# RichealYoung/BRIEF_PyTorch

Measured on AMD Instinct MI355X. Metric: encode_voxels_per_sec, higher is better.
Workload: dtype f32; 1 GPU; SingleTask 512^3 synthetic uint16 volume, SIREN 4x256 (layers=5, features=256, w0=20), randompoint sample_size=100000, datal2, Adamax lr=1e-3; layers=5, features=256, sample_size=100000, params=198657

## Files before the change

### brief_pytorch_amd/csrc/brief_hip.hip

```cpp
#include <hip/hip_runtime.h>
#include <hip/hip_ext.h>
#include <stdint.h>
#include <stdio.h>
#include <string.h>
#include <stdlib.h>
#include <mutex>
#include "brief_layout.h"
#include "brief_math.h"

#include "brief_device.inc"
#include "brief_fused.inc"
#include "brief_lean.inc"
#include "brief_wide.inc"
#include "brief_small.inc"
#include "brief_wgrad.inc"
#include "brief_x3.inc"
#include "brief_reduce.inc"
#include "brief_bf16.inc"
#include "brief_aux.inc"
#include "brief_ffn.inc"
#include "brief_nerf.inc"
#include "brief_mfn.inc"

static thread_local char g_err[512] = "";
// ... 829 lines not shown
            const int lds_big = (int)(sizeof(float) * 4 * W16B_PANEL);
            if (int rc = dev_attr_once((const void *)k_wgrad16_big, lds_big)) return rc;
            if (ov.on) {
                wa.kb_lo = 0; wa.kb_hi = ov.kb_body; wa.split_lo = 0; wa.nsplit_here = ov.na;
                hipLaunchKernelGGL(k_wgrad16_big, dim3((hidden * ov.na + 7) / 8 * 8 * 4), dim3(512), lds_big, st, wa);
                wa.kb_lo = ov.kb_body; wa.kb_hi = np / 64; wa.split_lo = ov.na; wa.nsplit_here = 1;
                hipLaunchKernelGGL(k_wgrad16_big, dim3((hidden + 7) / 8 * 8 * 4), dim3(512), lds_big, side, wa);
            } else {
                const int groups8 = (hidden * nsp + 7) / 8 * 8;
                hipLaunchKernelGGL(k_wgrad16_big, dim3(groups8 * 4), dim3(512), lds_big, st, wa);
            }
        } else if (hidden > 0) {
            hipLaunchKernelGGL(k_wgrad16<false>, dim3(hidden * nb * nb * nsp), dim3(256), sizeof(float) * 4 * W16_PANEL, st, wa);
        }
        hipLaunchKernelGGL(k_wgrad16<true>, dim3((wa.bias_jobs ? hidden * nb * nsp : 0) + 2 * nb * nsp_s), dim3(256), sizeof(float) * 4 * W16_PANEL, side, wa);
        HIP_TRY(hipGetLastError());
        if (ov.on) {
            HIP_TRY(hipEventRecord(dev_state()->aux_join, side));
            HIP_TRY(hipStreamWaitEvent(st, dev_state()->aux_join, 0));
        }
        const int64_t l0c = (int64_t)d->features * d->cin + d->features;
        const int64_t hcnt = brief_canon_head_off(*d) - l0c;
        if (hidden > 0) {
            ReduceArgs ra;
            memset(&ra, 0, sizeof(ra));
            ra.d = *d; ra.slabs = ws + w16.slabs; ra.nsplit = nsp; ra.sgroups = 1;
            ra.grads = grads; ra.loss_out = loss_out; ra.inv_count = inv16;
            if (upd) { ra.update = 1; ra.opt = upd->opt; ra.params = upd->params; ra.s1 = upd->s1; ra.s2 = upd->s2; ra.pk = upd->pk; }
            ra.sgroups = 1;
            const int nbh = (int)((hcnt + 255) / 256);
            hipLaunchKernelGGL(k_reduce, dim3(nbh), dim3(256), 0, st, ra, nbh);
            HIP_TRY(hipGetLastError());
        }
        Reduce16Args r16;
        memset(&r16, 0, sizeof(r16));
        r16.d = *d; r16.slabs = ws + w16.slabs + (int64_t)hidden * nsp * (FP * FP + FP); r16.nsplit = nsp_s;
        r16.rec = fa.rec; r16.nwg = g16; r16.grads = grads; r16.loss_out = loss_out; r16.inv_count = inv16;
        if (upd) { r16.update = 1; r16.opt = upd->opt; r16.params = upd->params; r16.s1 = upd->s1; r16.s2 = upd->s2; r16.pk = upd->pk; }
        const int64_t items = l0c + (int64_t)d->cout * d->features + d->cout + 1;
        hipLaunchKernelGGL(k_reduce16, dim3((unsigned)((items + 3) / 4)), dim3(256), 0, st, r16);
        HIP_TRY(hipGetLastError());
        return 0;
    }
    const bool small = use_small(*d);
    const FusedPlan fp = fused_plan(*d, batch->n, true);
    TailPlan tp;
    memset(&tp, 0, sizeof(tp));
    if (!small) tp = fused_tail_plan(*d, batch->n);
    const int grid1 = small ? small_grid(*d, batch->n) : (tp.on ? tp.grid_body + tp.grid_tail : fp.grid);
    const int nsplit = small ? (d->layers > 2 ? grid1 : 0) : wgrad_splits(*d, batch->n);
    const float inv_count = (float)(1.0 / ((double)batch->n * d->cout));

    FusedArgs fa;
    memset(&fa, 0, sizeof(fa));
    fa.d = *d; fa.pk = packed;
    fa.coords = batch->coords; fa.targets = batch->targets; fa.weights = batch->weights;
    fa.idx = batch->idx; fa.offset = batch->offset; fa.n = batch->n;
    if (!batch->idx && batch->rng_pop > 0) { fa.rng_pop = (uint64_t)batch->rng_pop; fa.rng_seed = batch->rng_seed; fa.rng_step = batch->rng_step; }
    fill_grid(fa.grid, grid);
    fa.loss_kind = loss_kind; fa.thr = thr; fa.beta = beta; fa.inv_count = inv_count;
    fa.Z = ws + wl.z; fa.D = ws + wl.dd; fa.npad = brief_npad_d(*d, batch->n);
    fa.rec = ws + wl.rec; fa.slabs = brief_use_wide(*d) ? ws + wl.img : ws + wl.slabs; fa.yhat_out = yhat_out;
    fa.stagger_cus = kCUs; fa.stagger = g_stagger; fa.diag = g_diag;
    fa.pers_wgs = fp.pers_wgs; fa.pers_tiles = fp.pers_tiles;
    ReduceArgs ra;
    memset(&ra, 0, sizeof(ra));
    ra.d = *d; ra.rec = fa.rec; ra.nrec_wg = grid1; ra.slabs = ws + wl.slabs; ra.nsplit = nsplit;
    int sg_small = 8;
    while (sg_small < 32 && sg_small * 16 < nsplit) sg_small *= 2;
    if (g_reduce_sg_small > 0) sg_small = g_reduce_sg_small;
    ra.sgroups = small ? sg_small : g_reduce_sg_big;
    const int rthreads = 256;
    ra.grads = grads; ra.loss_out = loss_out; ra.inv_count = inv_count;
    if (upd) { ra.update = 1; ra.opt = upd->opt; ra.params = upd->params; ra.s1 = upd->s1; ra.s2 = upd->s2; ra.pk = upd->pk; }
    const int64_t l0_count = (int64_t)d->features * d->cin + d->features;
    const int64_t hcount = brief_canon_head_off(*d) - l0_count;
    const int64_t skinny = d->features + (int64_t)d->cout * ((d->features + 3) / 4) + 2;
    ra.vec = (!small && g_reduce_vec && d->precision == BRIEF_PREC_F32 && rthreads * 4 <= 1024) ? (d->features % 4 == 0 ? 4 : (d->features % 2 == 0 ? 2 : 0)) : 0;
    {
        const uintptr_t bits = (uintptr_t)grads | (uintptr_t)ra.params | (uintptr_t)ra.s1 | (uintptr_t)ra.s2 | (uintptr_t)ra.pk | (uintptr_t)ra.slabs;
        while (ra.vec > 1 && bits % (sizeof(float) * ra.vec) != 0) ra.vec /= 2;
        if (ra.vec == 1) ra.vec = 0;
    }
    const int ppb = rthreads / ra.sgroups * (ra.vec ? ra.vec : 1);
    const int nb_hidden = (int)((hcount + ppb - 1) / ppb);
    const int wpb = rthreads / 64;
    const int nb_skinny = (int)((skinny + wpb - 1) / wpb);
    if (plan_only) {
        if (!small) return fail(BRIEF_ERR_INVALID, "internal: step plans exist for narrow nets only");
        plan_only->fa = fa; plan_only->ra = ra; plan_only->grid1 = grid1; plan_only->nb_hidden = nb_hidden;
        plan_only->nb_reduce = nb_hidden + nb_skinny; plan_only->nt = nt; plan_only->hb = small_hb(*d);
        return 0;
    }
    const bool prof = prof_live();
    hipEvent_t pe0 = prof ? dev_state()->prof_ev[2 * g_prof_n] : nullptr, pe1 = prof ? dev_state()->prof_ev[2 * g_prof_n + 1] : nullptr;
    if (small) {
        const int hb = small_hb(*d);
#define BRIEF_CASE(NTV, HBV)                                                                                        \
    if (nt == NTV && hb == HBV)                                                                                     \
        launch_timed(k_small<NTV, HBV>, grid1, 256, sizeof(float) * SmallLds<NTV>::TOTAL, st, fa, pe0, pe1);
        BRIEF_CASE(1, 1) BRIEF_CASE(1, 3) BRIEF_CASE(1, 5) BRIEF_CASE(1, 7)
        BRIEF_CASE(2, 1) BRIEF_CASE(2, 3) BRIEF_CASE(2, 5) BRIEF_CASE(2, 7)
#undef BRIEF_CASE
        HIP_TRY(hipGetLastError());
    } else if (!tp.on) {
        if (int rc = launch_fused<true>(fa, grid1, st, pe0, pe1)) return rc;
    }
    hipStream_t side = st;
    if (tp.on) {
        DevState *ds = dev_state();
        if (!ds) return fail(BRIEF_ERR_INVALID, "out of host memory");
        if (!ds->aux2_init) {
            HIP_TRY(hipStreamCreateWithFlags(&ds->aux2, hipStreamNonBlocking));
            HIP_TRY(hipEventCreateWithFlags(&ds->aux2_fork, hipEventDisableTiming));
            HIP_TRY(hipEventCreateWithFlags(&ds->aux2_join, hipEventDisableTiming));
            ds->aux2_init = true;
        }
        side = ds->aux2;
        fa.n_begin = 0; fa.n_end = tp.tiles_body * 32; fa.rec_base = 0;
        fa.pers_wgs = tp.grid_body; fa.pers_tiles = tp.tiles_body;
        if (int rc = launch_fused<true>(fa, tp.grid_body, st, pe0, nullptr)) return rc;
        HIP_TRY(hipEventRecord(ds->aux2_fork, st));
        HIP_TRY(hipStreamWaitEvent(side, ds->aux2_fork, 0));
        fa.n_begin = tp.tiles_body * 32; fa.n_end = 0; fa.rec_base = tp.grid_body;
        fa.pers_wgs = 0;
        if (int rc = launch_fused<true>(fa, tp.grid_tail, st, nullptr, pe1)) return rc;
    }
    if (prof) ++g_prof_n;

    if (!small && nsplit > 0) {
        WgradArgs wa;
        memset(&wa, 0, sizeof(wa));
        wa.d = *d; wa.Z = fa.Z; wa.D = fa.D; wa.npad = fa.npad; wa.nsplit = nsplit; wa.slabs = ws + wl.slabs;
        wa.stamps = ws + wl.rec + rec_region_floats(*d) - 256 * 8 * 8;
        const int per_split = (d->layers - 2) * wgrad_nq(nt) * wgrad_nq(nt);
        if (tp.mode == 2) {
            wa.uneven = 1; wa.n_norm = tp.n_norm; wa.kfix_n = tp.kfix_n; wa.kfix_s = tp.kfix_s;
            wa.kb_lo = 0; wa.kb_hi = fa.npad / 32;
            wa.split_lo = 0; wa.nsplit_here = tp.n_norm;
            if (int rc = launch_wgrad(*d, wa, wa.nsplit_here * per_split, side)) return rc;
            wa.split_lo = tp.n_norm; wa.nsplit_here = nsplit - tp.n_norm;
            if (int rc = launch_wgrad(*d, wa, wa.nsplit_here * per_split, st)) return rc;
        } else {
            const int nsA = tp.on ? nsplit - 1 : nsplit;
            wa.kb_lo = 0; wa.kb_hi = tp.on ? tp.tiles_body : fa.npad / 32; wa.split_lo = 0; wa.nsplit_here = nsA;
            for (int part = 0; part < (tp.on ? 2 : 1); ++part) {
                if (part) { wa.kb_lo = tp.tiles_body; wa.kb_hi = fa.npad / 32; wa.split_lo = nsA; wa.nsplit_here = 1; }
                if (int rc = launch_wgrad(*d, wa, wa.nsplit_here * per_split, part || !tp.on ? st : side)) return rc;
            }
        }
    }
    if (tp.on) {
        HIP_TRY(hipEventRecord(dev_state()->aux2_join, side));
        HIP_TRY(hipStreamWaitEvent(st, dev_state()->aux2_join, 0));
    }
    if (g_reduce_part == 1) hipLaunchKernelGGL(k_reduce, dim3(nb_hidden), dim3(rthreads), 0, st, ra, nb_hidden);
    else if (g_reduce_part == 2) hipLaunchKernelGGL(k_reduce, dim3(nb_skinny), dim3(rthreads), 0, st, ra, 0);
    else hipLaunchKernelGGL(k_reduce, dim3(nb_hidden + nb_skinny), dim3(rthreads), 0, st, ra, nb_hidden);
    HIP_TRY(hipGetLastError());
    return 0;
}

extern "C" {

int brief_siren_train_step(const brief_siren_desc *d, const float *packed, const brief_grid_desc *grid,
                           const brief_batch_desc *batch, int loss_kind, float thr, float beta,
                           float *grads, float *loss_out, float *yhat_out,
                           void *workspace, int64_t workspace_bytes, void *stream)
// ... 1237 lines not shown
```

### brief_pytorch_amd/csrc/brief_reduce.inc

```
struct OptimScalars { int kind; float w1, fb2, w2, feps, nstep, bc2s; };

__device__ __forceinline__ float optim_rule(const OptimScalars &o, float gi, float p0, float &m, float &u)
{
    const int kind = o.kind;
    const float w1 = o.w1, fb2 = o.fb2, w2 = o.w2, feps = o.feps, nstep = o.nstep, bc2s = o.bc2s;
    if (kind == BRIEF_OPT_ADAMAX) {
        const float mn = __fmaf_rn(w1, __fsub_rn(gi, m), m);
        const float ua = __fmul_rn(u, fb2), ub = __fadd_rn(fabsf(gi), feps);
        const float un = ua > ub ? ua : ub;
        m = mn; u = un;
        return __fadd_rn(p0, __fdiv_rn(__fmul_rn(nstep, mn), un));
    } else if (kind == BRIEF_OPT_ADAM) {
        const float mn = __fmaf_rn(w1, __fsub_rn(gi, m), m);
        const float vn = __fadd_rn(__fmul_rn(u, fb2), __fmul_rn(w2, __fmul_rn(gi, gi)));
        m = mn; u = vn;
        const float den = __fadd_rn(__fdiv_rn(sqrtf(vn), bc2s), feps);
        return __fadd_rn(p0, __fdiv_rn(__fmul_rn(nstep, mn), den));
    }
    return __fadd_rn(p0, __fmul_rn(nstep, gi));
}

struct OptimPre { float p, m, u; };
__device__ __forceinline__ OptimPre optim_prefetch(const OptimScalars &o, const float *__restrict__ p, const float *__restrict__ s1,
                                                   const float *__restrict__ s2, int64_t i)
{
    OptimPre r;
    r.p = p[i];
    r.m = o.kind != BRIEF_OPT_SGD ? s1[i] : 0.f;
    r.u = o.kind != BRIEF_OPT_SGD ? s2[i] : 0.f;
    return r;
}
__device__ __forceinline__ float optim_commit(const OptimScalars &o, float gi, OptimPre pre, float *__restrict__ p, float *__restrict__ s1,
                                              float *__restrict__ s2, int64_t i)
{
    const float pn = optim_rule(o, gi, pre.p, pre.m, pre.u);
    if (o.kind != BRIEF_OPT_SGD) { s1[i] = pre.m; s2[i] = pre.u; }
    p[i] = pn;
    return pn;
}

__device__ __forceinline__ float optim_apply(const OptimScalars &o, float gi, float *__restrict__ p, float *__restrict__ s1,
                                             float *__restrict__ s2, int64_t i)
{
    return optim_commit(o, gi, optim_prefetch(o, p, s1, s2, i), p, s1, s2, i);
}

__global__ void k_optim(OptimScalars o, float *__restrict__ p, const float *__restrict__ g, float *__restrict__ s1,
                        float *__restrict__ s2, int64_t n)
{
    const int64_t i = (int64_t)blockIdx.x * blockDim.x + threadIdx.x;
    if (i >= n) return;
    optim_apply(o, g[i], p, s1, s2, i);
}

struct ReduceArgs {
    brief_siren_desc d;
    const float *rec;
    int nrec_wg;
    const float *slabs;
    int nsplit;
    int sgroups;
    int vec;
    float *grads;
    float *loss_out;
    float inv_count;
    int update;
    OptimScalars opt;
    float *params, *s1, *s2, *pk;
};

__device__ __forceinline__ int64_t frag_index(int NT, int row, int col)
{
    const int mt = row >> 5, ii = row & 31, kt = col >> 5, rem = col & 31;
    const int q = rem >> 3, hi = (rem >> 2) & 1, j = rem & 3;
    return ((((int64_t)mt * NT + kt) * 4 + q) * 64 + 32 * hi + ii) * 4 + j;
}

template <int V> struct ReduceVec;
template <> struct ReduceVec<2> { typedef float2 T; };
template <> struct ReduceVec<4> { typedef float4 T; };
template <int V>
__device__ __forceinline__ void reduce_hidden_vec(const ReduceArgs &a, const OptimScalars &opt, int bid, float *fold)
{
    typedef typename ReduceVec<V>::T VT;
    const brief_siren_desc &d = a.d;
    const int F = d.features, NT = brief_nt(d), FP = 32 * NT;
    const int64_t l0_count = (int64_t)F * d.cin + F;
    const int64_t hcount = brief_canon_head_off(d) - l0_count;
    const int SG = a.sgroups, ppb = (int)blockDim.x / SG;
    const int pl = threadIdx.x % ppb, sg = threadIdx.x / ppb;
    const int64_t hidx = ((int64_t)bid * ppb + pl) * V;
    const bool live = hidx < hcount;
    const int64_t per = (int64_t)F * F + F;
    const int l = live ? 1 + (int)(hidx / per) : 1;
    const int64_t r = live ? hidx % per : 0;
    float s[V], pp[V], pm[V], pu[V];
#pragma unroll
    for (int c = 0; c < V; ++c) { s[c] = 0.f; pp[c] = 0.f; pm[c] = 0.f; pu[c] = 0.f; }
    const bool mine = a.update && live && sg == 0;
    if (mine) {
        *reinterpret_cast<VT *>(pp) = *reinterpret_cast<const VT *>(a.params + l0_count + hidx);
        if (opt.kind != BRIEF_OPT_SGD) {
            *reinterpret_cast<VT *>(pm) = *reinterpret_cast<const VT *>(a.s1 + l0_count + hidx);
            *reinterpret_cast<VT *>(pu) = *reinterpret_cast<const VT *>(a.s2 + l0_count + hidx);
        }
    }
    if (live) {
        int64_t so;
        if (r < (int64_t)F * F) so = (r / F) * FP + (r % F);
        else so = (int64_t)FP * FP + (r - (int64_t)F * F);
        const int64_t slab_sz = (int64_t)FP * FP + FP;
        const float *base = a.slabs + (int64_t)(l - 1) * a.nsplit * slab_sz + so;
#pragma unroll 8
        for (int sp = sg; sp < a.nsplit; sp += SG) {
            float v[V];
            *reinterpret_cast<VT *>(v) = *reinterpret_cast<const VT *>(base + (int64_t)sp * slab_sz);
#pragma unroll
            for (int c = 0; c < V; ++c) s[c] += v[c];
        }
    }
    if (SG > 1) {
        *reinterpret_cast<VT *>(fold + (int64_t)threadIdx.x * V) = *reinterpret_cast<VT *>(s);
        __syncthreads();
        if (sg == 0)
            for (int gq = 1; gq < SG; ++gq) {
                float v[V];
                *reinterpret_cast<VT *>(v) = *reinterpret_cast<const VT *>(fold + (int64_t)(gq * ppb + pl) * V);
#pragma unroll
                for (int c = 0; c < V; ++c) s[c] += v[c];
            }
    }
    if (!live || sg != 0) return;
    *reinterpret_cast<VT *>(a.grads + l0_count + hidx) = *reinterpret_cast<VT *>(s);
    if (!a.update) return;
    float pv[V];
#pragma unroll
    for (int c = 0; c < V; ++c) pv[c] = optim_rule(opt, s[c], pp[c], pm[c], pu[c]);
    if (opt.kind != BRIEF_OPT_SGD) {
        *reinterpret_cast<VT *>(a.s1 + l0_count + hidx) = *reinterpret_cast<VT *>(pm);
        *reinterpret_cast<VT *>(a.s2 + l0_count + hidx) = *reinterpret_cast<VT *>(pu);
    }
    *reinterpret_cast<VT *>(a.params + l0_count + hidx) = *reinterpret_cast<VT *>(pv);
    float *blk = a.pk + brief_pk_hidden(d, l);
    const float fs = brief_phase_scale(d, l), bs = brief_om_prev(d, l);
    float pf[V];
#pragma unroll
    for (int c = 0; c < V; ++c) pf[c] = fs * pv[c];
    if (r < (int64_t)F * F) {
        const int o = (int)(r / F), i = (int)(r % F);
        *reinterpret_cast<VT *>(blk + frag_index(NT, o, i)) = *reinterpret_cast<VT *>(pf);
#pragma unroll
        for (int c = 0; c < V; ++c) blk[(int64_t)FP * FP + frag_index(NT, i + c, o)] = bs * pv[c];
    } else {
        *reinterpret_cast<VT *>(blk + 2 * (int64_t)FP * FP + (r - (int64_t)F * F)) = *reinterpret_cast<VT *>(pf);
    }
}

__device__ __forceinline__ void reduce_body(const ReduceArgs &a, const OptimScalars &opt, float *loss_out, int nb_hidden, int bid)
{
    const brief_siren_desc &d = a.d;
    const int F = d.features, cin = d.cin, cout = d.cout;
    const int NT = brief_nt(d), FP = 32 * NT, WM = brief_wm(NT), WS = brief_ws(NT);
    const int64_t off_head = brief_canon_head_off(d);
    const int64_t l0_count = (int64_t)F * cin + F;
    if (bid < nb_hidden) {
        __shared__ __attribute__((aligned(16))) float fold[1024];
        if (a.vec == 4) { reduce_hidden_vec<4>(a, opt, bid, fold); return; }
        if (a.vec == 2) { reduce_hidden_vec<2>(a, opt, bid, fold); return; }
        const int64_t hcount = off_head - l0_count;
        const int SG = a.sgroups, ppb = (int)blockDim.x / SG;
        const int pl = threadIdx.x % ppb, sg = threadIdx.x / ppb;
        const int64_t hidx = (int64_t)bid * ppb + pl;
        const bool live = hidx < hcount;
        const int64_t per = (int64_t)F * F + F;
        const int l = live ? 1 + (int)(hidx / per) : 1;
        const int64_t r = live ? hidx % per : 0;
        float s = 0.f;
        OptimPre pre = {0.f, 0.f, 0.f};
        if (a.update && live && sg == 0) pre = optim_prefetch(opt, a.params, a.s1, a.s2, l0_count + hidx);
        if (live) {
            int64_t so;
            if (r < (int64_t)F * F) so = (r / F) * FP + (r % F);
            else so = (int64_t)FP * FP + (r - (int64_t)F * F);
            const int64_t slab_sz = (int64_t)FP * FP + FP;
            const float *base = a.slabs + (int64_t)(l - 1) * a.nsplit * slab_sz + so;
            if (SG >= 16) {
#pragma unroll 16
                for (int sp = sg; sp < a.nsplit; sp += SG) s += base[(int64_t)sp * slab_sz];
            } else {
#pragma unroll 8
                for (int sp = sg; sp < a.nsplit; sp += SG) s += base[(int64_t)sp * slab_sz];
            }
        }
        if (SG > 1) {
            fold[threadIdx.x] = s;
            __syncthreads();
            if (sg == 0)
                for (int gq = 1; gq < SG; ++gq) s += fold[gq * ppb + pl];
        }
        if (!live || sg != 0) return;
        a.grads[l0_count + hidx] = s;
        if (a.update) {
            const float pv = optim_commit(opt, s, pre, a.params, a.s1, a.s2, l0_count + hidx);
            float *blk = a.pk + brief_pk_hidden(d, l);
            if (r < (int64_t)F * F) {
                const int o = (int)(r / F), i = (int)(r % F);
                const float pf = brief_phase_scale(d, l) * pv, pb = brief_om_prev(d, l) * pv;
                if (d.precision != BRIEF_PREC_BF16) {
                    blk[frag_index(NT, o, i)] = pf;
                    blk[(int64_t)FP * FP + frag_index(NT, i, o)] = pb;
                }
                if (d.precision == BRIEF_PREC_BF16X3) {
                    uint16_t *h16 = reinterpret_cast<uint16_t *>(a.pk + brief_pk16_off(d, l));
                    uint16_t *l16 = reinterpret_cast<uint16_t *>(a.pk + brief_pk16_off(d, l) + brief_pk16_region(d));
                    uint16_t fh, fl, bh, bl;
                    x3_split_f16(BRIEF_X3_FWD_SCALE * pf, fh, fl);
                    x3_split_bf16(pb, bh, bl);
                    h16[brief_frag16_index(NT, o, i)] = fh;
                    h16[(int64_t)FP * FP + brief_frag16_index(NT, i, o)] = bh;
                    l16[brief_frag16_index(NT, o, i)] = fl;
                    l16[(int64_t)FP * FP + brief_frag16_index(NT, i, o)] = bl;
                } else if (d.precision == BRIEF_PREC_BF16) {
                    __bf16 *b16 = reinterpret_cast<__bf16 *>(a.pk + brief_pk16_off(d, l));
                    b16[brief_frag16_index(NT, o, i)] = (__bf16)pf;
                    b16[(int64_t)FP * FP + brief_frag16_index(NT, i, o)] = (__bf16)pb;
                }
            } else {
                blk[2 * (int64_t)FP * FP + (r - (int64_t)F * F)] = brief_phase_scale(d, l) * pv;
            }
        }
        return;
    }
    const int lane = threadIdx.x & 63;
    const int64_t grp = (int64_t)(bid - nb_hidden) * (blockDim.x >> 6) + (threadIdx.x >> 6);
    const int Fq = (F + 3) >> 2;
    const int64_t g_head = F, g_bias = g_head + (int64_t)cout * Fq, g_loss = g_bias + 1;
    const int nrec = a.nrec_wg * WS;
    const int TR = brief_rec_tr(NT), rec_floats = brief_rec_floats(NT);
    if (grp > g_loss) return;
    int slot, wmo = 0;
    int64_t e_par = -1;
    if (grp < g_head) {
        const int o = (int)grp;
        slot = (((o >> 5) / WM) * 32 + (o & 31)) * 4;
        wmo = (o >> 5) % WM;
        if (lane < cin) e_par = (int64_t)o * cin + lane;
        else if (lane == 3) e_par = (int64_t)F * cin + o;
    } else if (grp < g_bias) {
        const int64_t r = grp - g_head;
// ... 76 lines not shown
```

### brief_pytorch_amd/csrc/brief_wgrad.inc

```
struct WgradArgs {
    brief_siren_desc d;
    const float *Z;
    const float *D;
    int64_t npad;
    int nsplit;
    int64_t kb_lo, kb_hi;
    int split_lo, nsplit_here;
    int uneven, n_norm;
    int64_t kfix_n, kfix_s;
    float *slabs;
    float *stamps;
};

constexpr int wgrad_nq(int NT) { return (NT + 7) / 8; }
constexpr int wgrad_qt(int NT) { return (NT + wgrad_nq(NT) - 1) / wgrad_nq(NT); }
#ifndef BRIEF_WGRAD_XSPLIT
#define BRIEF_WGRAD_XSPLIT 1
#endif
#ifndef BRIEF_WGRAD_LIST
#define BRIEF_WGRAD_LIST(QT) ((QT) == 3 || (QT) == 5)
#endif
#ifndef BRIEF_WGRAD_STAGE_BIAS
#define BRIEF_WGRAD_STAGE_BIAS 1
#endif
#ifndef BRIEF_WGRAD_FRAG_PIPE
#define BRIEF_WGRAD_FRAG_PIPE 1
#endif
#ifndef BRIEF_WGRAD_FRAG_PIPE2
#define BRIEF_WGRAD_FRAG_PIPE2 1
#endif
constexpr int wgrad_wmk(int QT) { return QT >= 2 ? 2 : 1; }
constexpr int wgrad_wnk(int QT) { return QT >= 7 ? 4 : (QT >= 2 ? 2 : 1); }
constexpr bool wgrad_list(int QT) { return BRIEF_WGRAD_LIST(QT); }
constexpr int wgrad_wk(int QT) { return QT >= 7 || wgrad_list(QT) ? 1 : (QT >= 2 ? 2 : 4); }
constexpr int wgrad_lds_floats(int NT)
{
    const int QT = wgrad_qt(NT);
    const int WMk = wgrad_wmk(QT), WNk = wgrad_wnk(QT), WK = wgrad_wk(QT);
    const int NWv = WMk * WNk, TN = (QT + WNk - 1) / WNk;
    const int fold = (WK - 1) * NWv * TN * 1024 + (WK - 1) * NWv * 64, panels = 4 * 32 * QT * 36;
    return fold > panels ? fold : panels;
}

template <int NT, int QTR = 0>
__global__ __launch_bounds__(512, 2) void k_wgrad(const WgradArgs a)
{
    constexpr bool RTW = NT == 0;
    const int nt_w = RTW ? brief_nt(a.d) : NT;
    const int FP = 32 * nt_w;
    const int NQ = RTW ? (nt_w + 7) / 8 : wgrad_nq(NT);
    constexpr int QT = RTW ? QTR : wgrad_qt(NT), QP = 32 * QT;
    constexpr bool LIST = wgrad_list(QT);
    constexpr int LCNT = QT * QT / 8, LREM = QT * QT % 8;
    constexpr bool HET7 = QT == 7 && !LIST;
    constexpr bool XS = BRIEF_WGRAD_XSPLIT && (LIST || HET7) && QT * QT % 8 == 1;
    constexpr int XSLOT = LIST ? LCNT : 6;
    constexpr int WMk = HET7 || LIST ? 2 : wgrad_wmk(QT), WNk = HET7 || LIST ? 4 : wgrad_wnk(QT);
    constexpr int WK = wgrad_wk(QT);
    constexpr int NWv = WMk * WNk;
    constexpr int TM = HET7 || LIST ? 1 : (QT + WMk - 1) / WMk, TN = LIST ? LCNT + (LREM ? 1 : 0) : (HET7 ? 7 : (QT + WNk - 1) / WNk);
    constexpr bool MEX = QT % WMk == 0, NEX = QT % WNk == 0;
    constexpr int LDSW = 36;
    constexpr int NLD = (QP * 8 + 511) / 512;
    constexpr int PANEL = QP * LDSW;
    constexpr bool FULL = (QP * 8) % 512 == 0;
    extern __shared__ __attribute__((aligned(16))) float smem[];

    const int tid = threadIdx.x;
    const int lane = tid & 63;
    const int wave = __builtin_amdgcn_readfirstlane(tid >> 6);
    const int hi = lane >> 5, ln = lane & 31;
    const int wk = wave / NWv, wrem = wave % NWv;
    const int wmk = wrem / WNk, wnk = wrem % WNk;
    const bool kactive = wk < WK;
    const int quad = blockIdx.x % (NQ * NQ), bsl = blockIdx.x / (NQ * NQ);
    const int qm = quad / NQ, qn = quad % NQ;
    const bool uneven = RTW && a.uneven;
    const int hidden_l = a.d.layers - 2;
    const int l = uneven ? 1 + bsl % hidden_l : 1 + bsl / a.nsplit_here;
    const int split = uneven ? bsl / hidden_l : bsl % a.nsplit_here;
    const int64_t nchunks = a.kb_hi - a.kb_lo;
    int64_t c0 = a.kb_lo + nchunks * split / a.nsplit_here, c1 = a.kb_lo + nchunks * (split + 1) / a.nsplit_here;
    if (uneven) {
        const int g0 = a.split_lo + split, g1 = g0 + 1;
        c0 = (g0 <= a.n_norm ? g0 * a.kfix_n : a.n_norm * a.kfix_n + (g0 - a.n_norm) * a.kfix_s) >> 16;
        c1 = g1 >= a.nsplit ? a.kb_hi : ((g1 <= a.n_norm ? g1 * a.kfix_n : a.n_norm * a.kfix_n + (g1 - a.n_norm) * a.kfix_s) >> 16);
    }
    const float *Dl = a.D + (int64_t)(l - 1) * FP * a.npad + qm * QP * 32;
    const float *Zl = a.Z + (int64_t)(l - 1) * FP * a.npad + qn * QP * 32;

    f32x16 acc[TM][TN];
    float dbacc[TM];
#pragma unroll
    for (int i = 0; i < TM; ++i) {
        dbacc[i] = 0.f;
#pragma unroll
        for (int jn = 0; jn < TN; ++jn)
#pragma unroll
            for (int r = 0; r < 16; ++r) acc[i][jn][r] = 0.f;
    }
    float dbl[LIST ? TN : 1];
    int lmt[LIST ? TN : 1], lnt[LIST ? TN : 1];
    if (LIST) {
        const int first = XS ? wave * LCNT : wave * LCNT + (wave > 8 - LREM ? wave - (8 - LREM) : 0);
#pragma unroll
        for (int k = 0; k < TN; ++k) {
            const int t = first + k < QT * QT ? first + k : QT * QT - 1;
            lmt[k] = t / QT; lnt[k] = t % QT; dbl[k] = 0.f;
        }
    }
    constexpr bool SBIAS = BRIEF_WGRAD_STAGE_BIAS && QT == 8;
    const bool want_bias = SBIAS && qn == 0;
    float bsum[NLD];
#pragma unroll
    for (int i = 0; i < NLD; ++i) bsum[i] = 0.f;
    float4 ra[NLD], rb[NLD];
    const int panel_bytes = (int)((int64_t)FP * a.npad * 4) - (RTW ? 0 : (NQ - 1) * QP * 128);
    const int rows_m = RTW ? FP - qm * QP : QP, rows_n = RTW ? FP - qn * QP : QP;
    const __amdgpu_buffer_rsrc_t rsD = __builtin_amdgcn_make_buffer_rsrc((void *)Dl, 0, panel_bytes, 0x00020000);
    const __amdgpu_buffer_rsrc_t rsZ = __builtin_amdgcn_make_buffer_rsrc((void *)Zl, 0, panel_bytes, 0x00020000);
    int voffs[NLD];
#pragma unroll
    for (int i = 0; i < NLD; ++i) {
        const int e = tid + 512 * i;
        voffs[i] = e * 16;
    }
#define WG_ISSUE(cc)                                                                              \
    _Pragma("unroll") for (int i = 0; i < NLD; ++i) {                                             \
        const int e = tid + 512 * i;                                                              \
        ra[i] = make_float4(0.f, 0.f, 0.f, 0.f);                                                  \
        rb[i] = make_float4(0.f, 0.f, 0.f, 0.f);                                                  \
        if (FULL || e < QP * 8) {                                                                 \
            if (!RTW || (e >> 3) < rows_m) ra[i] = bload4w(rsD, voffs[i], (int)((cc) * (FP * 128)));     \
            if (!RTW || (e >> 3) < rows_n) rb[i] = bload4w(rsZ, voffs[i], (int)((cc) * (FP * 128)));     \
        }                                                                                         \
    }
#define WG_STAGE_A(buf, i)                                                                        \
    {                                                                                             \
        const int e = tid + 512 * (i);                                                            \
        if (FULL || e < QP * 8)                                                                   \
            *reinterpret_cast<float4 *>(smem + (buf) * 2 * PANEL + (e >> 3) * LDSW + (e & 7) * 4) = ra[i]; \
    }
#define WG_STAGE_B(buf, i)                                                                        \
    {                                                                                             \
        const int e = tid + 512 * (i);                                                            \
        if (FULL || e < QP * 8) {                                                                 \
            float4 h;                                                                             \
            h.x = BRIEF_SIN_REV(rb[i].x); h.y = BRIEF_SIN_REV(rb[i].y);    \
            h.z = BRIEF_SIN_REV(rb[i].z); h.w = BRIEF_SIN_REV(rb[i].w);                           \
            *reinterpret_cast<float4 *>(smem + (buf) * 2 * PANEL + PANEL + (e >> 3) * LDSW + (e & 7) * 4) = h; \
        }                                                                                         \
    }
#define WG_BIAS_M(i, cm_) { bsum[i] = __fmaf_rn((cm_), (ra[i].x + ra[i].y) + (ra[i].z + ra[i].w), bsum[i]); }
#define WG_BIAS(i) WG_BIAS_M(i, 1.0f)
    WG_ISSUE(c0)
#pragma unroll
    for (int i = 0; i < NLD; ++i) { WG_STAGE_A(0, i) WG_STAGE_B(0, i) }
    if (want_bias) {
#pragma unroll
        for (int i = 0; i < NLD; ++i) WG_BIAS(i)
    }
    {
        const int64_t cn = c0 + 1 < c1 ? c0 + 1 : c1 - 1;
        WG_ISSUE(cn)
    }
    lds_barrier();
#ifdef BRIEF_STAMPS
    float st_acc[10] = {0.f, 0.f, 0.f, 0.f, 0.f, 0.f, 0.f, 0.f, 0.f, 0.f};
    long long st_last = clock64();
#endif
    if constexpr (LIST || HET7) {
    auto chunk_loop = [&](auto role_c) __attribute__((always_inline)) {
    constexpr int ROLE = decltype(role_c)::value;
    for (int64_t c = c0; c < c1; ++c) {
        const int cur = (int)(c - c0) & 1;
        const float *As = smem + cur * 2 * PANEL, *Bs = As + PANEL;
        const float cm_l = want_bias && c + 1 < c1 ? 1.0f : 0.0f;
        STAMP(0)
        if constexpr (LIST) {
            constexpr int CNT = XS ? LCNT : LCNT + ROLE;
#pragma unroll
            for (int gq = 0; gq < 4; ++gq) {
#pragma unroll
                for (int k = 0; k < CNT; ++k) {
                    const float4 a_ = *reinterpret_cast<const float4 *>(As + (32 * lmt[k] + ln) * LDSW + 8 * gq + 4 * hi);
                    const float4 b_ = *reinterpret_cast<const float4 *>(Bs + (32 * lnt[k] + ln) * LDSW + 8 * gq + 4 * hi);
                    if (!SBIAS) dbl[k] += (a_.x + a_.y) + (a_.z + a_.w);
                    acc[0][k] = MFMA(a_.x, b_.x, acc[0][k]); acc[0][k] = MFMA(a_.y, b_.y, acc[0][k]);
                    acc[0][k] = MFMA(a_.z, b_.z, acc[0][k]); acc[0][k] = MFMA(a_.w, b_.w, acc[0][k]);
                }
                if (XS && gq == ROLE) {
                    const float4 a_ = *reinterpret_cast<const float4 *>(As + (32 * (QT - 1) + ln) * LDSW + 8 * gq + 4 * hi);
                    const float4 b_ = *reinterpret_cast<const float4 *>(Bs + (32 * (QT - 1) + ln) * LDSW + 8 * gq + 4 * hi);
                    acc[0][XSLOT] = MFMA(a_.x, b_.x, acc[0][XSLOT]); acc[0][XSLOT] = MFMA(a_.y, b_.y, acc[0][XSLOT]);
                    acc[0][XSLOT] = MFMA(a_.z, b_.z, acc[0][XSLOT]); acc[0][XSLOT] = MFMA(a_.w, b_.w, acc[0][XSLOT]);
                }
                if (gq >= 2) {
#pragma unroll
                    for (int i = 0; i < NLD; ++i)
                        if ((i & 1) == (gq & 1)) { WG_STAGE_A(cur ^ 1, i) WG_STAGE_B(cur ^ 1, i) if (SBIAS) WG_BIAS_M(i, cm_l) }
                }
            }
        } else if constexpr (HET7) {
#define WG_FRAG(P, row) (*reinterpret_cast<const float4 *>((P) + (32 * (row) + ln) * LDSW + 8 * gq + 4 * hi))
#define WG_MFMA4(k, A_, B_) { acc[0][k] = MFMA((A_).x, (B_).x, acc[0][k]); acc[0][k] = MFMA((A_).y, (B_).y, acc[0][k]); \
                              acc[0][k] = MFMA((A_).z, (B_).z, acc[0][k]); acc[0][k] = MFMA((A_).w, (B_).w, acc[0][k]); }
#define WG_STAGE_NEXT                                                                   \
            if (gq >= 2) {                                                              \
                _Pragma("unroll") for (int i = 0; i < NLD; ++i)                         \
                    if ((i & 1) == (gq & 1)) { WG_STAGE_A(cur ^ 1, i) WG_STAGE_B(cur ^ 1, i) if (SBIAS) WG_BIAS_M(i, cm_l) } \
            }
            if constexpr (XS ? ROLE < 5 : ROLE == 0) {
#pragma unroll
                for (int gq = 0; gq < 4; ++gq) {
                    const float4 a_ = WG_FRAG(As, wave);
                    if (!SBIAS) dbacc[0] += (a_.x + a_.y) + (a_.z + a_.w);
#pragma unroll
                    for (int jn = 0; jn < 6; ++jn) {
                        const float4 b_ = WG_FRAG(Bs, jn);
                        WG_MFMA4(jn, a_, b_)
                    }
                    if (XS && gq == ROLE) {
                        const float4 a6 = WG_FRAG(As, 6), b6 = WG_FRAG(Bs, 6);
                        WG_MFMA4(6, a6, b6)
                    }
                    WG_STAGE_NEXT
                }
            } else {
#pragma unroll
                for (int gq = 0; gq < 4; ++gq) {
                    const float4 b6 = WG_FRAG(Bs, 6);
#pragma unroll
                    for (int i = 0; i < (XS ? 6 : 7); ++i) {
                        const float4 a_ = WG_FRAG(As, i);
                        WG_MFMA4(i, a_, b6)
                    }
                    WG_STAGE_NEXT
                }
            }
#undef WG_FRAG
#undef WG_MFMA4
#undef WG_STAGE_NEXT
        }
        STAMP(1)
        {
            const int64_t cn = c + 2 < c1 ? c + 2 : c1 - 1, cn1 = c + 1 < c1 ? c + 1 : c1 - 1;
            WG_ISSUE(cn)
        }
        STAMP(2)
        lds_barrier();
        STAMP(3)
    }
// ... 40 lines not shown
            }                                                                                                          \
        }
#define WG_MFMAS(AF, BF)                                                                                               \
        {                                                                                                              \
            _Pragma("unroll") for (int i = 0; i < TM; ++i) {                                                           \
                _Pragma("unroll") for (int jn = 0; jn < TN; ++jn) {                                                    \
                    if ((MEX || wmk * TM + i < QT) && (NEX || wnk * TN + jn < QT)) {                                   \
                        acc[i][jn] = MFMA(AF[i].x, BF[jn].x, acc[i][jn]);                                              \
                        acc[i][jn] = MFMA(AF[i].y, BF[jn].y, acc[i][jn]);                                              \
                        acc[i][jn] = MFMA(AF[i].z, BF[jn].z, acc[i][jn]);                                              \
                        acc[i][jn] = MFMA(AF[i].w, BF[jn].w, acc[i][jn]);                                              \
                    }                                                                                                  \
                }                                                                                                      \
            }                                                                                                          \
        }
#define WG_STAGE_NEXT(gq_)                                                                                             \
        if ((gq_) >= 2) {                                                                                              \
            _Pragma("unroll") for (int i = 0; i < NLD; ++i)                                                            \
                if ((i & 1) == ((gq_) & 1)) {                                                                          \
                    WG_STAGE_A(cur ^ 1, i) WG_STAGE_B(cur ^ 1, i)                                                      \
                    if (SBIAS) WG_BIAS_M(i, cm_r)                                                                      \
                }                                                                                                      \
        }
        if constexpr (BRIEF_WGRAD_FRAG_PIPE && WK == 1 && QT == 8) {
            float4 af0[TM], bf0[TN], af1[TM], bf1[TN];
            WG_READ_FRAGS(0, af0, bf0)
            WG_READ_FRAGS(1, af1, bf1)
            __builtin_amdgcn_sched_barrier(0);
            WG_MFMAS(af0, bf0)
            WG_READ_FRAGS(2, af0, bf0)
            __builtin_amdgcn_sched_barrier(0);
            WG_MFMAS(af1, bf1)
            WG_READ_FRAGS(3, af1, bf1)
            __builtin_amdgcn_sched_barrier(0);
            WG_MFMAS(af0, bf0)
            WG_STAGE_NEXT(2)
            WG_MFMAS(af1, bf1)
            WG_STAGE_NEXT(3)
        } else if constexpr (BRIEF_WGRAD_FRAG_PIPE2 && WK == 2 && QT >= 4) {
            float4 af0[TM], bf0[TN], af1[TM], bf1[TN];
            WG_READ_FRAGS(wk, af0, bf0)
            WG_READ_FRAGS(wk + 2, af1, bf1)
            __builtin_amdgcn_sched_barrier(0);
#pragma unroll
            for (int i = 0; i < TM; ++i)
                if (wnk == 0) {
                    dbacc[i] += (af0[i].x + af0[i].y) + (af0[i].z + af0[i].w);
                    dbacc[i] += (af1[i].x + af1[i].y) + (af1[i].z + af1[i].w);
                }
            WG_MFMAS(af0, bf0)
            WG_STAGE_NEXT(2)
            WG_MFMAS(af1, bf1)
            WG_STAGE_NEXT(3)
        } else {
#pragma unroll
        for (int gq = 0; gq < 4; ++gq) {
            if (kactive && (WK == 1 || (gq % WK) == wk)) {
                float4 af[TM], bf[TN];
                WG_READ_FRAGS(gq, af, bf)
                if (!SBIAS) {
#pragma unroll
                    for (int i = 0; i < TM; ++i)
                        if (wnk == 0) dbacc[i] += (af[i].x + af[i].y) + (af[i].z + af[i].w);
                }
                WG_MFMAS(af, bf)
            }
            WG_STAGE_NEXT(gq)
        }
        }
#undef WG_READ_FRAGS
#undef WG_MFMAS
#undef WG_STAGE_NEXT
        STAMP(1)
        {
            const int64_t cn = c + 2 < c1 ? c + 2 : c1 - 1, cn1 = c + 1 < c1 ? c + 1 : c1 - 1;
            WG_ISSUE(cn)
        }
        STAMP(2)
        lds_barrier();
        STAMP(3)
    }
    }
#ifdef BRIEF_STAMPS
    if (lane == 0 && a.stamps) for (int i = 0; i < 4; ++i) a.stamps[((int64_t)blockIdx.x * 8 + wave) * 8 + i] = st_acc[i];
#endif
#undef WG_ISSUE
#undef WG_STAGE_A
#undef WG_STAGE_B
#undef WG_BIAS
#undef WG_BIAS_M
    if (WK > 1) {
        float *red = smem;
        float *redb = smem + (WK - 1) * NWv * TN * 1024;
#pragma unroll
        for (int i = 0; i < TM; ++i) {
            if (i > 0) lds_barrier();
            if (kactive && wk > 0) {
#pragma unroll
                for (int jn = 0; jn < TN; ++jn)
#pragma unroll
                    for (int r = 0; r < 16; ++r)
                        red[(((wk - 1) * NWv + wrem) * TN + jn) * 1024 + r * 64 + lane] = acc[i][jn][r];
                redb[((wk - 1) * NWv + wrem) * 64 + lane] = dbacc[i];
            }
            lds_barrier();
            if (wk == 0) {
                for (int w = 1; w < WK; ++w) {
#pragma unroll
                    for (int jn = 0; jn < TN; ++jn)
#pragma unroll
                        for (int r = 0; r < 16; ++r)
                            acc[i][jn][r] += red[(((w - 1) * NWv + wrem) * TN + jn) * 1024 + r * 64 + lane];
                    dbacc[i] += redb[((w - 1) * NWv + wrem) * 64 + lane];
                }
            }
        }
    }
    float *slab = a.slabs + ((int64_t)(l - 1) * a.nsplit + a.split_lo + split) * ((int64_t)FP * FP + FP);
    if (want_bias) {
#pragma unroll
        for (int i = 0; i < NLD; ++i) {
            const int e = tid + 512 * i;
            if (FULL || e < QP * 8) {
                float v = bsum[i];
                v += __shfl_xor(v, 1); v += __shfl_xor(v, 2); v += __shfl_xor(v, 4);
                if ((tid & 7) == 0 && (e >> 3) < rows_m) slab[(int64_t)FP * FP + qm * QP + (e >> 3)] = v;
            }
        }
    }
    if (wk != 0) return;
    if (LIST) {
        const int cnt = XS ? LCNT + (wave == 0 ? 1 : 0) : LCNT + (LREM > 0 && wave >= 8 - LREM ? 1 : 0);
#pragma unroll
        for (int k = 0; k < TN; ++k) {
            if (k >= cnt) break;
            const int mt = XS && k == LCNT ? QT - 1 : lmt[k], nt = XS && k == LCNT ? QT - 1 : lnt[k];
            if ((!RTW || qm * QT + mt < nt_w) && (!RTW || qn * QT + nt < nt_w)) {
#pragma unroll
                for (int r = 0; r < 16; ++r)
                    slab[(int64_t)(qm * QP + 32 * mt + ROWMAP(r, hi)) * FP + qn * QP + 32 * nt + ln] = acc[0][k][r];
            }
            if (!SBIAS && qn == 0 && nt == 0 && !(XS && k == LCNT)) {
                const float tot = dbl[k] + __shfl_xor(dbl[k], 32);
                if (hi == 0 && (!RTW || qm * QT + mt < nt_w)) slab[(int64_t)FP * FP + qm * QP + 32 * mt + ln] = tot;
            }
        }
        return;
    }
    if (HET7) {
#pragma unroll
        for (int k = 0; k < 7; ++k) {
            int mt = wave < 7 ? wave : k, nt = wave < 7 ? k : 6;
            if (XS) {
                if (k == 6) { if (wave != 0) continue; mt = 6; nt = 6; }
            } else if (wave < 7 && k == 6) continue;
            if ((!RTW || qm * QT + mt < nt_w) && (!RTW || qn * QT + nt < nt_w)) {
#pragma unroll
                for (int r = 0; r < 16; ++r)
                    slab[(int64_t)(qm * QP + 32 * mt + ROWMAP(r, hi)) * FP + qn * QP + 32 * nt + ln] = acc[0][k][r];
            }
        }
        if (!SBIAS && qn == 0 && wave < 7) {
            const float tot = dbacc[0] + __shfl_xor(dbacc[0], 32);
            if (hi == 0 && (!RTW || qm * QT + wave < nt_w)) slab[(int64_t)FP * FP + qm * QP + 32 * wave + ln] = tot;
        }
        return;
    }
#pragma unroll
    for (int i = 0; i < TM; ++i) {
        const int mt = wmk * TM + i;
        if (mt < QT && (!RTW || qm * QT + mt < nt_w)) {
#pragma unroll
            for (int jn = 0; jn < TN; ++jn) {
                const int nt = wnk * TN + jn;
                if (nt < QT && (!RTW || qn * QT + nt < nt_w)) {
#pragma unroll
                    for (int r = 0; r < 16; ++r)
                        slab[(int64_t)(qm * QP + 32 * mt + ROWMAP(r, hi)) * FP + qn * QP + 32 * nt + ln] = acc[i][jn][r];
                }
            }
            if (!SBIAS && wnk == 0 && qn == 0) {
                const float tot = dbacc[i] + __shfl_xor(dbacc[i], 32);
                if (hi == 0) slab[(int64_t)FP * FP + qm * QP + 32 * mt + ln] = tot;
            }
        }
    }
}
```

Before: 101.8 million voxels/s.

## Store wgrad partial slabs in fragment-native layout and reduce them permuted

When NT==8, the weight-gradient kernel now writes its accumulator tiles to the split slabs as contiguous float4 chunks in MFMA fragment order, replacing per-element scattered row-major stores. A new hidden-layer reduce path reads these permuted slabs with float4 loads, maps each unit back to (row, col), and applies the optimizer plus packed-weight writes. The aim is coalesced slab writes in the wgrad epilogue, paid for by strided parameter/state accesses and a more complex index mapping in the reduce. Extra stamp instrumentation is added under a debug macro.

```diff
diff --git a/brief_pytorch_amd/csrc/brief_hip.hip b/brief_pytorch_amd/csrc/brief_hip.hip
--- a/brief_pytorch_amd/csrc/brief_hip.hip
+++ b/brief_pytorch_amd/csrc/brief_hip.hip
@@ -935,8 +935,10 @@
         while (ra.vec > 1 && bits % (sizeof(float) * ra.vec) != 0) ra.vec /= 2;
         if (ra.vec == 1) ra.vec = 0;
     }
+    ra.perm = !small && d->precision == BRIEF_PREC_F32 && wgrad_pslab(nt) ? 1 : 0;
     const int ppb = rthreads / ra.sgroups * (ra.vec ? ra.vec : 1);
-    const int nb_hidden = (int)((hcount + ppb - 1) / ppb);
+    const int64_t perm_units = (int64_t)(d->layers - 2) * (32 * nt * 32 * nt + 32 * nt) / 4;
+    const int nb_hidden = ra.perm ? (int)((perm_units + rthreads / ra.sgroups - 1) / (rthreads / ra.sgroups)) : (int)((hcount + ppb - 1) / ppb);
     const int wpb = rthreads / 64;
     const int nb_skinny = (int)((skinny + wpb - 1) / wpb);
     if (plan_only) {
diff --git a/brief_pytorch_amd/csrc/brief_reduce.inc b/brief_pytorch_amd/csrc/brief_reduce.inc
--- a/brief_pytorch_amd/csrc/brief_reduce.inc
+++ b/brief_pytorch_amd/csrc/brief_reduce.inc
@@ -61,6 +61,7 @@
     int nsplit;
     int sgroups;
     int vec;
+    int perm;
     float *grads;
     float *loss_out;
     float inv_count;
@@ -156,6 +157,90 @@
     }
 }
 
+__device__ __forceinline__ void reduce_hidden_perm(const ReduceArgs &a, const OptimScalars &opt, int bid, float *fold)
+{
+    const brief_siren_desc &d = a.d;
+    const int F = d.features, NT = brief_nt(d), FP = 32 * NT;
+    const int64_t l0_count = (int64_t)F * d.cin + F;
+    const int hidden = d.layers - 2;
+    const int SG = a.sgroups, ppb = (int)blockDim.x / SG;
+    const int pl = threadIdx.x % ppb, sg = threadIdx.x / ppb;
+    const int wunits = FP * FP / 4, units = wunits + FP / 4;
+    const int64_t ug = (int64_t)bid * ppb + pl;
+    const bool in_range = ug < (int64_t)hidden * units;
+    const int l = in_range ? 1 + (int)(ug / units) : 1;
+    const int u = in_range ? (int)(ug % units) : 0;
+    const bool is_w = u < wunits;
+    const int tile = u >> 8, lane = u & 63;
+    const int row0 = is_w ? 32 * (tile / NT) + 8 * ((u >> 6) & 3) + 4 * (lane >> 5) : 4 * (u - wunits);
+    const int col = is_w ? 32 * (tile % NT) + (lane & 31) : 0;
+    const bool live = in_range && col < F && row0 < F;
+    const int64_t per = (int64_t)F * F + F;
+    const int64_t e0 = l0_count + (int64_t)(l - 1) * per + (is_w ? (int64_t)row0 * F + col : (int64_t)F * F + row0);
+    const int64_t estep = is_w ? F : 1;
+    float s[4], pp[4], pm[4], pu[4];
+#pragma unroll
+    for (int c = 0; c < 4; ++c) { s[c] = 0.f; pp[c] = 0.f; pm[c] = 0.f; pu[c] = 0.f; }
+    const bool mine = a.update && live && sg == 0;
+    if (mine) {
+#pragma unroll
+        for (int c = 0; c < 4; ++c)
+            if (row0 + c < F) {
+                pp[c] = a.params[e0 + c * estep];
+                if (opt.kind != BRIEF_OPT_SGD) { pm[c] = a.s1[e0 + c * estep]; pu[c] = a.s2[e0 + c * estep]; }
+            }
+    }
+    if (live) {
+        const int64_t slab_sz = (int64_t)FP * FP + FP;
+        const float *base = a.slabs + (int64_t)(l - 1) * a.nsplit * slab_sz + 4 * (int64_t)u;
+#pragma unroll 8
+        for (int sp = sg; sp < a.nsplit; sp += SG) {
+            const float4 v = *reinterpret_cast<const float4 *>(base + (int64_t)sp * slab_sz);
+            s[0] += v.x; s[1] += v.y; s[2] += v.z; s[3] += v.w;
+        }
+    }
+    if (SG > 1) {
+        *reinterpret_cast<float4 *>(fold + (int64_t)threadIdx.x * 4) = make_float4(s[0], s[1], s[2], s[3]);
+        __syncthreads();
+        if (sg == 0)
+            for (int gq = 1; gq < SG; ++gq) {
+                const float4 v = *reinterpret_cast<const float4 *>(fold + (int64_t)(gq * ppb + pl) * 4);
+                s[0] += v.x; s[1] += v.y; s[2] += v.z; s[3] += v.w;
+            }
+    }
+    if (!live || sg != 0) return;
+#pragma unroll
+    for (int c = 0; c < 4; ++c)
+        if (row0 + c < F) a.grads[e0 + c * estep] = s[c];
+    if (!a.update) return;
+    float pv[4];
+#pragma unroll
+    for (int c = 0; c < 4; ++c) {
+        pv[c] = 0.f;
+        if (row0 + c < F) {
+            pv[c] = optim_rule(opt, s[c], pp[c], pm[c], pu[c]);
+            if (opt.kind != BRIEF_OPT_SGD) { a.s1[e0 + c * estep] = pm[c]; a.s2[e0 + c * estep] = pu[c]; }
+            a.params[e0 + c * estep] = pv[c];
+        }
+    }
+    float *blk = a.pk + brief_pk_hidden(d, l);
+    const float fs = brief_phase_scale(d, l), bs = brief_om_prev(d, l);
+    if (is_w) {
+        const int64_t bt = (int64_t)FP * FP + frag_index(NT, col, row0);
+        if (row0 + 3 < F) *reinterpret_cast<float4 *>(blk + bt) = make_float4(bs * pv[0], bs * pv[1], bs * pv[2], bs * pv[3]);
+#pragma unroll
+        for (int c = 0; c < 4; ++c)
+            if (row0 + c < F) {
+                blk[frag_index(NT, row0 + c, col)] = fs * pv[c];
+                if (row0 + 3 >= F) blk[bt + c] = bs * pv[c];
+            }
+    } else {
+#pragma unroll
+        for (int c = 0; c < 4; ++c)
+            if (row0 + c < F) blk[2 * (int64_t)FP * FP + row0 + c] = fs * pv[c];
+    }
+}
+
 __device__ __forceinline__ void reduce_body(const ReduceArgs &a, const OptimScalars &opt, float *loss_out, int nb_hidden, int bid)
 {
     const brief_siren_desc &d = a.d;
@@ -165,6 +250,7 @@
     const int64_t l0_count = (int64_t)F * cin + F;
     if (bid < nb_hidden) {
         __shared__ __attribute__((aligned(16))) float fold[1024];
+        if (a.perm) { reduce_hidden_perm(a, opt, bid, fold); return; }
         if (a.vec == 4) { reduce_hidden_vec<4>(a, opt, bid, fold); return; }
         if (a.vec == 2) { reduce_hidden_vec<2>(a, opt, bid, fold); return; }
         const int64_t hcount = off_head - l0_count;
diff --git a/brief_pytorch_amd/csrc/brief_wgrad.inc b/brief_pytorch_amd/csrc/brief_wgrad.inc
--- a/brief_pytorch_amd/csrc/brief_wgrad.inc
+++ b/brief_pytorch_amd/csrc/brief_wgrad.inc
@@ -29,6 +29,10 @@
 #ifndef BRIEF_WGRAD_FRAG_PIPE2
 #define BRIEF_WGRAD_FRAG_PIPE2 1
 #endif
+#ifndef BRIEF_WGRAD_PSLAB
+#define BRIEF_WGRAD_PSLAB 1
+#endif
+constexpr bool wgrad_pslab(int NT) { return BRIEF_WGRAD_PSLAB && BRIEF_WGRAD_STAGE_BIAS && NT == 8; }
 constexpr int wgrad_wmk(int QT) { return QT >= 2 ? 2 : 1; }
 constexpr int wgrad_wnk(int QT) { return QT >= 7 ? 4 : (QT >= 2 ? 2 : 1); }
 constexpr bool wgrad_list(int QT) { return BRIEF_WGRAD_LIST(QT); }
@@ -66,6 +70,9 @@
     constexpr bool FULL = (QP * 8) % 512 == 0;
     extern __shared__ __attribute__((aligned(16))) float smem[];
 
+#ifdef BRIEF_STAMPS
+    const long long st_t0 = clock64(), st_w0 = wall_clock64();
+#endif
     const int tid = threadIdx.x;
     const int lane = tid & 63;
     const int wave = __builtin_amdgcn_readfirstlane(tid >> 6);
@@ -168,6 +175,7 @@
 #ifdef BRIEF_STAMPS
     float st_acc[10] = {0.f, 0.f, 0.f, 0.f, 0.f, 0.f, 0.f, 0.f, 0.f, 0.f};
     long long st_last = clock64();
+    st_acc[4] = (float)(st_last - st_t0);
 #endif
     if constexpr (LIST || HET7) {
     auto chunk_loop = [&](auto role_c) __attribute__((always_inline)) {
@@ -374,7 +382,8 @@
     }
     }
 #ifdef BRIEF_STAMPS
-    if (lane == 0 && a.stamps) for (int i = 0; i < 4; ++i) a.stamps[((int64_t)blockIdx.x * 8 + wave) * 8 + i] = st_acc[i];
+    const long long st_le = clock64();
+    if (lane == 0 && a.stamps) for (int i = 0; i < 5; ++i) a.stamps[((int64_t)blockIdx.x * 8 + wave) * 8 + i] = st_acc[i];
 #endif
 #undef WG_ISSUE
 #undef WG_STAGE_A
@@ -458,6 +467,17 @@
         }
         return;
     }
+    if constexpr (wgrad_pslab(NT)) {
+        float4 *dst = reinterpret_cast<float4 *>(slab) + lane;
+#pragma unroll
+        for (int i = 0; i < TM; ++i)
+#pragma unroll
+            for (int jn = 0; jn < TN; ++jn)
+#pragma unroll
+                for (int g = 0; g < 4; ++g)
+                    dst[(((wmk * TM + i) * NT + wnk * TN + jn) * 4 + g) * 64] =
+                        make_float4(acc[i][jn][4 * g], acc[i][jn][4 * g + 1], acc[i][jn][4 * g + 2], acc[i][jn][4 * g + 3]);
+    } else {
 #pragma unroll
     for (int i = 0; i < TM; ++i) {
         const int mt = wmk * TM + i;
@@ -477,4 +497,13 @@
             }
         }
     }
+    }
+#ifdef BRIEF_STAMPS
+    asm volatile("s_waitcnt vmcnt(0)" ::: "memory");
+    if (lane == 0 && a.stamps) {
+        const long long t1 = clock64();
+        float *sp = a.stamps + ((int64_t)blockIdx.x * 8 + wave) * 8;
+        sp[5] = (float)(t1 - st_le); sp[6] = (float)(t1 - st_t0); sp[7] = (float)(wall_clock64() - st_w0);
+    }
+#endif
 }
```

Measured after the change: 101.7 million voxels/s (median of 3 runs). Within noise of the previous version (-0.1%).
